# lym01803/FinalProject-LosslessImageCompression

Measured on AMD Instinct MI355X. Metric: encode+decode Mpixels/s (imagenet64, bit-exact round trip), higher is better.
Workload: dtype f32

## Files before the change

### finalproject-losslessimagecompression_amd/csrc/conv3_dx3.hip

```cpp
#include <hip/hip_runtime.h>
#include <stdint.h>
#include <stdlib.h>
#include <string.h>

#include <type_traits>
#include <utility>

#include "idf_cdf.h"
#include "idf_codec_internal.h"
#include "wino_common.h"

#pragma clang fp contract(off)

namespace idf {

typedef float d4 __attribute__((ext_vector_type(4)));
typedef _Float16 e4 __attribute__((ext_vector_type(4)));
typedef _Float16 e8 __attribute__((ext_vector_type(8)));
typedef unsigned int v4u __attribute__((ext_vector_type(4)));
typedef __bf16 b8 __attribute__((ext_vector_type(8)));

struct Dx3Args {
  const uint16_t* xs;
  int64_t P;
// ... 44 lines not shown
#ifndef IDF_DX3_SB
#define IDF_DX3_SB 1
#endif
#ifndef IDF_DX3_DMA0
#define IDF_DX3_DMA0 0
#endif
#ifndef IDF_DX3_DMAS
#define IDF_DX3_DMAS 1
#endif
#ifndef IDF_DX3_STAG
#define IDF_DX3_STAG 0
#endif
#ifndef IDF_DX3_STAMPS
#define IDF_DX3_STAMPS 0
#endif
#ifndef IDF_DX3_STAMP_BLOCK
#define IDF_DX3_STAMP_BLOCK 100
#endif
#if IDF_DX3_STAMPS
__device__ unsigned long long g_dx3_stamp[8][40][4];
__device__ unsigned long long g_dx3_phase[8][6];
#define DX3_PHASE(j, v)                                                                      \
  do {                                                                                      \
    if (blockIdx.x == IDF_DX3_STAMP_BLOCK && lane == 0) g_dx3_phase[wave][(j)] = (v);       \
  } while (0)
#define DX3_STAMP(slab, j)                                                                 \
  do {                                                                                    \
    if (blockIdx.x == IDF_DX3_STAMP_BLOCK && (slab) < 40 && lane == 0)                    \
      g_dx3_stamp[wave][(slab)][(j)] = __builtin_amdgcn_s_memtime();                      \
  } while (0)
#else
#define DX3_STAMP(slab, j) do { } while (0)
#define DX3_PHASE(j, v) do { } while (0)
#endif
#ifndef IDF_DX3_TL
#define IDF_DX3_TL 0
#endif
#if IDF_DX3_TL
__device__ unsigned long long g_dx3_tl[4096][8];
#define DX3_TL(j)                                                                          \
  do {                                                                                    \
    if (tid == 0 && blockIdx.x < 4096) g_dx3_tl[blockIdx.x][(j)] = __builtin_amdgcn_s_memrealtime(); \
  } while (0)
__device__ unsigned long long g_dx3_tlml[1024][16][4];
#define DX3_TLML(li, j)                                                                    \
  do {                                                                                    \
    if (ML && tid == 0 && blockIdx.x < 1024 && (li) < 16)                                 \
      g_dx3_tlml[blockIdx.x][(li)][(j)] = __builtin_amdgcn_s_memrealtime();               \
  } while (0)
#else
#define DX3_TL(j) do { } while (0)
#define DX3_TLML(li, j) do { } while (0)
#endif
#ifndef IDF_DX3_KSPLIT
#define IDF_DX3_KSPLIT 4
#endif
#ifndef IDF_DX3_KSPLIT16
#define IDF_DX3_KSPLIT16 1
#endif
#ifndef IDF_DX3_TWO_MIN
#define IDF_DX3_TWO_MIN 512
#endif
#ifndef IDF_DX3_FORCE1
#define IDF_DX3_FORCE1 0
#endif

#ifndef IDF_DX3_PAIRS
#define IDF_DX3_PAIRS 0
#endif
#ifndef IDF_DX3_PRIO
#define IDF_DX3_PRIO 0
#endif
#ifndef IDF_DX3_PRIO_K
#define IDF_DX3_PRIO_K 4
#endif
#ifndef IDF_DX3_MIX
#define IDF_DX3_MIX 0
#endif
#ifndef IDF_DX3_WAVES
#define IDF_DX3_WAVES 8
#endif
constexpr int kDxWaves = IDF_DX3_WAVES;
constexpr int kDxThreads = 64 * kDxWaves;
constexpr uint32_t kDxInvalid = 0xFFFFFFF0u;
constexpr uint32_t kDxOff = 0x80000000u;
constexpr float kDxInGuard = 32768.0f;
constexpr float kDxOutGuard = 8192.0f;

template <int NF, int WR, int PITCH, int PLANE_KIB, bool BF>
struct Dx3Lds {
  static constexpr int T = WR * kDxWaves / 16;
  static constexpr int HR = WR + 2;
  static constexpr int NS = BF ? 2 * HR - 1 : IDF_DX3_PAIRS ? 3 * HR - 1 + 2 * WR : 5 * HR - 1;
  static constexpr int NPL = BF ? 1 : 2;
  static constexpr int PLANE = PLANE_KIB * 1024;
  static constexpr int SLOTS = PLANE / 32;
  static constexpr int WOFF = T * NPL * PLANE;
  static constexpr int WPART = 9 * NF * 512;
  static constexpr int WST = BF ? (WPART + 1023) / 1024 * 1024 : 2 * WPART;
  static constexpr int STAGE = WOFF + WST;
  static constexpr int ZOFF = 2 * STAGE;
  static constexpr int BOFF = ZOFF + NF * 512;
  static constexpr int HOFF = BOFF + 16 * NF * 16 * 4;
  static constexpr int FOFF = HOFF + 16 * NF * 16 * 4;
  static constexpr int BYTES = FOFF + 16;
  static constexpr int HPIECES = T * NPL * PLANE_KIB;
// ... 80 lines not shown
#pragma unroll
      for (int cls = 0; cls < 16; ++cls) {
        float v = bt[0];
        if (Ly.vtap) {
#pragma unroll
          for (int tap = 0; tap < 9; ++tap) {
            const int dy = tap / 3 - 1, dx = tap % 3 - 1;
            const bool ok = !((dy < 0 && (cls & 1)) || (dy > 0 && (cls & 2)) ||
                              (dx < 0 && (cls & 4)) || (dx > 0 && (cls & 8)));
            v = ok ? v + bt[1 + tap] : v;
          }
          v = cls == 0 ? bt[10] : v;
        }
        btab[cls * NN + tid] = n < g.N ? v : 0.0f;
      }
    }
    if (g.nh > 0) {
#pragma unroll
      for (int i = 0; i < HPER; ++i) {
        const int e = tid + i * kDxThreads, o = e / NN, hn = grp * NN + e - o * NN;
        if (e < NE) htab[e] = (o < g.nh && hn < g.N) ? ht[i] : 0.0f;
      }
    }
  }
};

template <int NF, int WR, int PITCH, int PLANE_KIB, bool BF, bool ML, int WRW = WR>
__device__ __forceinline__ void dx3_block(const Dx3Args& g, const Dx3MLArgs* ml, char* lds) {
  using L = Dx3Lds<NF, WR, PITCH, PLANE_KIB, BF>;
  constexpr bool MIX = WRW != WR;
  constexpr int T = L::T, HR = WRW + 2;
  constexpr int NS = BF ? 2 * HR - 1 : IDF_DX3_PAIRS ? 3 * HR - 1 + 2 * WRW : 5 * HR - 1;
  static_assert(!MIX || (T == 2 && kDxWaves == 8 && !ML && (WRW == WR + 1 || WRW == WR - 1)),
                "mixed rows: two tiles of two SIMD pairs, per-layer launches");
  static_assert(L::WST % 1024 == 0, "weight stage must be whole 1-KiB DMA pieces");
  static_assert(L::BYTES <= 160 * 1024, "LDS");
  static_assert(HR >= 3, "the A-fragment reads of a phase take its last three steps");
  static_assert(IDF_DX3_DMAS == 0 || IDF_DX3_DMA0 + IDF_DX3_STAG + (L::PPW - 1) * IDF_DX3_DMAS < NS,
                "every DMA piece of a slab is issued within the slab's steps");
  int* last_flag = (int*)(lds + L::FOFF);
  const int tid = threadIdx.x, lane = tid & 63;
  const int wave = __builtin_amdgcn_readfirstlane(tid >> 6);
  const int bid = xcd_contiguous(blockIdx.x, gridDim.x);
  const int per_chunk = g.ngroup * g.nblk_tiles;
  const int chunk = udiv_s(bid, per_chunk);
  const int rem = bid - chunk * per_chunk;
  const int grp = udiv_s(rem, g.nblk_tiles);
  const int tb = rem - grp * g.nblk_tiles;
  const int tw = MIX ? (wave & 3) >> 1 : wave / (kDxWaves / T);
  constexpr int WR_OLD = IDF_DX3_MIX == 2 ? WR - 1 : WR + 1;
  const int r0 = MIX ? 2 * WR * (wave & 1) + ((wave & 4) ? WR_OLD : 0) : WR * (wave % (kDxWaves / T));
  d4 hreg[WRW];
  const int nlayers = ML ? ml->nlayers : 1;
  for (int li = 0; li < nlayers; ++li) {
  int tid_o = tid, lane_o = lane, wave_o = wave, tb_o = tb, tw_o = tw, r0_o = r0, grp_o = grp,
      chunk_o = chunk;
  if constexpr (ML) {
    asm volatile("" : "+v"(tid_o), "+v"(lane_o), "+v"(wave_o), "+v"(tb_o), "+v"(tw_o), "+v"(r0_o),
                 "+v"(grp_o), "+v"(chunk_o));
    wave_o = __builtin_amdgcn_readfirstlane(wave_o);
    tb_o = __builtin_amdgcn_readfirstlane(tb_o);
    tw_o = __builtin_amdgcn_readfirstlane(tw_o);
    r0_o = __builtin_amdgcn_readfirstlane(r0_o);
    grp_o = __builtin_amdgcn_readfirstlane(grp_o);
    chunk_o = __builtin_amdgcn_readfirstlane(chunk_o);
  }
  const int tid = tid_o, lane = lane_o, wave = wave_o, tb = tb_o, tw = tw_o, r0 = r0_o,
            grp = grp_o, chunk = chunk_o;
  const int lz = 0;
  DX3_TLML(li, 0);
  Dx3Layer Ly;
  if constexpr (ML) {
    Ly = ml->layer[li];
  } else {
    Ly = Dx3Layer{g.Wt, g.b3, g.vtap, g.bfull, g.out, g.yscale, g.C, g.nslab, g.nchunk,
                  g.chunk_slabs, g.hlast};
  }
  const int tile = tb * T + tw + lz;

  const int64_t plane_b = g.P * 32;
  const int xs_rec = (int)(g.xs_slab < (int64_t)kDxInvalid ? g.xs_slab : (int64_t)kDxInvalid);
  uint32_t pbase[L::PPW];
  int plo[L::PPW];
  bool pok[L::PPW];
  const int s0 = ML ? 0 : chunk * Ly.chunk_slabs;
  const int s1 = ML ? Ly.nslab : min(Ly.nslab, s0 + Ly.chunk_slabs);
  const uint32_t wslab = (uint32_t)(g.ngroup * L::WST);
  const int64_t wbytes = (int64_t)Ly.nslab * wslab;
  const __amdgpu_buffer_rsrc_t wr = __builtin_amdgcn_make_buffer_rsrc(
      (void*)Ly.Wt, 0, (int)(wbytes < (int64_t)kDxInvalid ? wbytes : (int64_t)kDxInvalid), 0x00020000);
  auto dma = [&](int s, int st, int i) {
    if (!pok[i]) return;
    const bool halo = i < L::PH;
    if (halo ? (IDF_DX3_ABLATE & 1) : (IDF_DX3_ABLATE & 4)) return;
    const __amdgpu_buffer_rsrc_t xr = __builtin_amdgcn_make_buffer_rsrc(
        (void*)((const char*)g.xs + (int64_t)s * g.xs_slab), 0, xs_rec, 0x00020000);
    const uint32_t off = pbase[i] + (halo ? 0u : (uint32_t)(s * g.ngroup) * (uint32_t)L::WST);
    __builtin_amdgcn_raw_ptr_buffer_load_lds(halo ? xr : wr,
                                             (dx_lds_ptr_t)(lds + st * L::STAGE + plo[i]), 16,
                                             off, 0, 0, 0);
  };
#pragma unroll
  for (int i = L::PH; i < L::PPW; ++i) {
    const int k = wave + kDxWaves * (i - L::PH);
    pok[i] = k < L::WPIECES;
    plo[i] = pok[i] ? L::WOFF + k * 1024 : 0;
    pbase[i] = pok[i] ? (uint32_t)(grp * L::WST + k * 1024 + lane * 16) : kDxOff;
    if (s1 > s0) dma(s0, 0, i);
  }
  uint32_t forg[T] = {};
  int fu0[T] = {}, fy0[T] = {};
  if constexpr (PITCH == 18) if (g.fastplan) {
#pragma unroll
    for (int t = 0; t < T; ++t) {
      const int tt = tb * T + t;
      const DxTile dtt = dx_tile(g, tt < g.ntiles ? tt : 0);
      const bool tok = tt < g.ntiles && dtt.band < g.B;
      fu0[t] = __builtin_amdgcn_readfirstlane(dtt.u0 - 1);
      fy0[t] = __builtin_amdgcn_readfirstlane(tok ? dtt.u0y - 1 : INT32_MIN / 2);
      forg[t] = __builtin_amdgcn_readfirstlane(
          ((uint32_t)dtt.band * (uint32_t)g.H + (uint32_t)(dtt.u0y - 1)) * (uint32_t)g.Wd + (uint32_t)(dtt.u0 - 1));
    }
  }
#pragma unroll
  for (int i = 0; i < L::PH; ++i) {
    const int k = wave + kDxWaves * i;
    pok[i] = k < L::HPIECES;
    pbase[i] = kDxOff;
    plo[i] = 0;
    if (pok[i]) {
      const int t = k / (L::NPL * PLANE_KIB), pl = (k / PLANE_KIB) % L::NPL, pi = k % PLANE_KIB;
      plo[i] = (t * L::NPL + pl) * L::PLANE + pi * 1024;
      const int slot = 32 * pi + (lane >> 1);
      const int tt = tb * T + t;
      bool fast = false;
      if constexpr (PITCH == 18) fast = g.fastplan != 0;
      if (fast) {
        const int cr = slot / PITCH, cc = slot - cr * PITCH;
        int u0m = fu0[0], y0m = fy0[0];
        uint32_t org = forg[0];
#pragma unroll
        for (int u = 1; u < T; ++u)
          if (t == u) { u0m = fu0[u]; y0m = fy0[u]; org = forg[u]; }
        const bool ok = (uint32_t)(u0m + cc) < (uint32_t)g.Wd && (uint32_t)(y0m + cr) < (uint32_t)g.H &&
                        cr < PITCH;
        if (ok)
          pbase[i] = (uint32_t)pl * (uint32_t)plane_b +
                     (org + (uint32_t)cr * (uint32_t)g.Wd + (uint32_t)cc) * (uint32_t)g.xs_pix +
                     (uint32_t)((lane & 1) * 16);
      } else if (tt < g.ntiles) {
        const DxTile dt = dx_tile(g, tt);
        int ix, x, iy, y;
        bool ok;
        if (g.gut) {
          const int cr = slot / PITCH, cc = slot - cr * PITCH;
          const int u = dt.u0 - 1 + cc, uy = dt.u0y - 1 + cr;
          ix = u >= 0 ? udiv_s(u, g.wp) : 0;
          x = u >= 0 ? u - ix * g.wp : -1;
          iy = uy >= 0 ? udiv_s(uy, g.hp) : 0;
          y = uy >= 0 ? uy - iy * g.hp : -1;
          ok = cr < g.ch && cc < g.segw;
        } else {
          const int sk = g.seg ? udiv_s(slot, g.seg) : 0;
          const int rr = slot - sk * g.seg;
          const int cr = rr / PITCH, cc = rr - cr * PITCH;
          ok = sk < g.nseg && cc < g.segw && cr < g.ch;
          ix = dt.ix0 + sk;
          x = (sk ? 0 : dt.xf0) - 1 + cc;
          const int vy = dt.vy0 + cr;
          iy = udiv_s(vy, g.H + 2);
          y = vy - iy * (g.H + 2) - 1;
        }
        const int b = (dt.band * g.nby + iy) * g.nbx + ix;
        ok = ok && x >= 0 && x < g.Wd && ix < g.nbx && y >= 0 && y < g.H && iy < g.nby && b < g.B;
        if (ok)
          pbase[i] = (uint32_t)(pl * plane_b + ((((int64_t)b * g.H + y) * g.Wd + x) * g.xs_pix) + (lane & 1) * 16);
      }
    }
    if (s1 > s0) dma(s0, 0, i);
  }
  DX3_TL(0);
  if (!ML || li == 0)
    for (int e = tid; e < NF * 512 / 16; e += kDxThreads) *(d4*)(lds + L::ZOFF + 16 * e) = d4{0.f, 0.f, 0.f, 0.f};
  DX3_PHASE(0, __builtin_amdgcn_s_memtime());
  DX3_PHASE(4, __builtin_amdgcn_s_memrealtime());

  const int j = lane & 15, q = lane >> 4;
  const DxTile dt = dx_tile(g, tile < g.ntiles ? tile : 0);
  const int jx = g.xskip ? 3 * (j >> 1) + (j & 1) : j;
  const int uj = dt.u0 + jx;
  const int pw = g.gut ? g.wp : g.Wd;
  const int ixj = udiv_s(uj, pw);
  const int xj = uj - ixj * pw;
  const int kj = ixj - dt.ix0;
  const int colb = g.gut ? jx : kj * g.seg + (kj ? j - (ixj * g.Wd - dt.u0) : j);
  const int uyw = dt.u0y + r0;
  int iyw = udiv_s(uyw, g.H);
  if (iyw > g.nby - 1) iyw = g.nby - 1;
  const int rowb = g.gut ? r0 : uyw + 2 * iyw - dt.vy0;

  const int slot0 = rowb * PITCH + colb;
  const int tb0 = tw * L::NPL * L::PLANE;
  const int oP = tb0 + (q >> 1) * L::PLANE + slot0 * 32 + (q & 1) * 16;
  const int oF = tb0 + slot0 * 32 + (q & 1) * 16 + (q >> 1) * 32;
  const int oG = tb0 + slot0 * 32 + (q & 1) * 16 + 64 + (q >> 1) * PITCH * 32;
  const int oAH = L::WOFF + j * 32 + (q & 1) * 16;
  constexpr int WLO = BF ? 0 : L::WPART;
  const int oAF = L::WOFF + WLO + j * 32 + (q & 1) * 16 + (q >> 1) * NF * 512;
  const int oAG = L::WOFF + WLO + 2 * NF * 512 + j * 32 + (q & 1) * 16 + (q >> 1) * 3 * NF * 512;
  const int oAO = L::WOFF + WLO + 8 * NF * 512 + j * 32 + (q & 1) * 16;
  const int oAHF = L::WOFF + j * 32 + (q & 1) * 16 + (q >> 1) * NF * 512;
  const int oAHG = L::WOFF + 2 * NF * 512 + j * 32 + (q & 1) * 16 + (q >> 1) * 3 * NF * 512;
  const bool zlane = q < 2;
  const char* zO = lds + L::ZOFF + j * 32 + (q & 1) * 16;

  if constexpr (ML) if (li == 0) {
#pragma unroll
    for (int m = 0; m < WRW; ++m) hreg[m] = d4{0.f, 0.f, 0.f, 0.f};
    if (g.nh > 0) {
      const bool lane_ok0 = xj < g.Wd && ixj < g.nbx;
#pragma unroll
      for (int m = 0; m < WRW; ++m) {
        int iy = iyw, y = uyw + m - iyw * g.H;
        if (g.gut) {
          iy = udiv_s(uyw + m, g.hp);
          y = uyw + m - iy * g.hp;
        }
        const int img = (dt.band * g.nby + iy) * g.nbx + ixj;
        const bool ok = lane_ok0 && y < g.H && iy < g.nby && img < g.B;
        if (ok && 4 * q < g.nh) {
          const float* xr = ml->hx + (((int64_t)img * g.H + y) * g.Wd + xj) * ml->hld_x;
          d4 h;
#pragma unroll
          for (int i = 0; i < 4; ++i) h[i] = 4 * q + i < g.nh ? ml->hb[4 * q + i] : 0.0f;
          for (int c = 0; c < ml->hc0; c += 4) {
            const d4 xv = *(const d4*)(xr + c);
#pragma unroll
            for (int i = 0; i < 4; ++i) {
              const int o = 4 * q + i;
              if (o < g.nh) {
                const d4 wv = *(const d4*)(g.hw + (int64_t)o * g.ldhw + c);
#pragma unroll
                for (int k = 0; k < 4; ++k) h[i] = __builtin_fmaf(wv[k], xv[k], h[i]);
              }
            }
          }
          hreg[m] = h;
        }
      }
    }
  }

  Dx3Tables<NF> tabs;
  DX3_PHASE(1, __builtin_amdgcn_s_memtime());
  DX3_TL(1);


  d4 acc[WRW][NF];
#pragma unroll
  for (int m = 0; m < WRW; ++m)
#pragma unroll
    for (int n = 0; n < NF; ++n) acc[m][n] = d4{0.f, 0.f, 0.f, 0.f};

  auto rd = [](const char* p) { return *(const e8*)p; };
  auto mma = [](const e8& a, const e8& bb, d4& c) {
    if (IDF_DX3_ABLATE & 16) c[0] += (float)(a[0] * bb[0]);
    else if constexpr (BF)
      c = __builtin_amdgcn_mfma_f32_16x16x32_bf16(__builtin_bit_cast(b8, a), __builtin_bit_cast(b8, bb),
                                                   c, 0, 0, 0);
    else c = __builtin_amdgcn_mfma_f32_16x16x32_f16(a, bb, c, 0, 0, 0);
  };
  auto rdB = [&](const char* p) -> e8 {
    if (IDF_DX3_ABLATE & 32) return e8{(_Float16)1, (_Float16)(lane & 7), 0, 0, 0, 0, 0, (_Float16)(p == nullptr)};
    return rd(p);
  };
  auto rdA = [&](const char* p) -> e8 {
    if (IDF_DX3_ABLATE & 64) return e8{(_Float16)2, (_Float16)(lane & 3), 0, 0, 0, 0, 0, (_Float16)(p == nullptr)};
    return rd(p);
  };

  constexpr int DB = IDF_DX3_DB, RB = DB + 1;
  e8 Bq[RB];
  e8 AS[2][3][NF];
  e8 AZ[2][NF];
  auto read_B = [&](const char* st, int t) -> e8 {
    if (t < 3 * HR) return rdB(st + oP + ((t % HR) * PITCH + t / HR) * 32);
    if (t < 4 * HR) return rdB(st + oF + (t - 3 * HR) * PITCH * 32);
    return rdB(st + oG + (t - 4 * HR) * PITCH * 32);
  };
  auto read_A = [&](const char* st, int p, int dy, e8 (&A)[NF]) {
#pragma unroll
    for (int n = 0; n < NF; ++n)
      A[n] = p < 3 ? rdA(st + oAH + ((dy * 3 + p) * NF + n) * 512)
                   : rdA(st + oAF + (3 * dy * NF + n) * 512);
  };
  auto mma_rows = [&](const e8 (&A)[3][NF], const e8& Bv, int h) {
#pragma unroll
    for (int dy = 0; dy < 3; ++dy) {
      const int m = h - dy;
      if (m < 0 || m >= WRW) continue;
#pragma unroll
      for (int n = 0; n < NF; ++n) mma(A[dy][n], Bv, acc[m][n]);
    }
  };

  for (int s = s0; s < s1; ++s) {
    const char* cur = lds + ((s - s0) & 1) * L::STAGE;
    DX3_STAMP(s - s0, 0);
    asm volatile("s_waitcnt vmcnt(0) lgkmcnt(0)" ::: "memory");
    if (!(IDF_DX3_ABLATE & 8)) __builtin_amdgcn_s_barrier();
    DX3_STAMP(s - s0, 1);
    if (s == s0) DX3_TL(2);
    if (s == s0) DX3_TLML(li, 1);
    if (s == s0) tabs.load(g, Ly, grp, tid);
    if (s == s0 + 1) tabs.store((float*)(lds + L::BOFF), (float*)(lds + L::HOFF), g, Ly, grp, tid);
    __builtin_amdgcn_sched_barrier(0);
    const bool more = s + 1 < s1;
    const int nst = (s + 1 - s0) & 1;
    auto dma_step = [&](auto tc) {
      constexpr int t = decltype(tc)::value;
      constexpr int ds = IDF_DX3_DMAS > 0 ? IDF_DX3_DMAS : 1;
      auto dma_at = [&](auto dtc) {
        constexpr int dt_ = decltype(dtc)::value;
        if constexpr (IDF_DX3_DMAS == 0 && dt_ == 0) {
          if (more) {
#pragma unroll
            for (int i = 0; i < L::PPW; ++i) dma(s + 1, nst, i);
          }
        } else if constexpr (IDF_DX3_DMAS > 0 && dt_ >= 0 && dt_ % ds == 0 && dt_ / ds < L::PPW) {
          if (more) dma(s + 1, nst, dt_ / ds);
        }
      };
      if (IDF_DX3_STAG == 0 || !(wave & 4)) dma_at(std::integral_constant<int, t - IDF_DX3_DMA0>{});
      else dma_at(std::integral_constant<int, t - IDF_DX3_DMA0 - IDF_DX3_STAG>{});
    };
    if constexpr (BF) {
      auto read_Bf = [&](const char* st, int t) -> e8 {
        if (t < HR) return rdB(st + oF + t * PITCH * 32);
        return rdB(st + oG + (t - HR) * PITCH * 32);
      };
#pragma unroll
      for (int k = 0; k < (DB > 3 ? DB : 3); ++k) {
        if (k < DB) Bq[k] = read_Bf(cur, k);
        if (k < 3) read_A(cur, 3, k, AS[1][k]);
      }
      auto stepb = [&](auto tc) {
        constexpr int t = decltype(tc)::value;
        if (IDF_DX3_SB) __builtin_amdgcn_sched_barrier(0);
        dma_step(tc);
        if constexpr (t == 1 || t == 2) {
#pragma unroll
          for (int n = 0; n < NF; ++n) {
            if (t == 1) AZ[0][n] = rdA(cur + oAG + n * 512);
            else AZ[1][n] = rdA(zlane ? zO + n * 512 : cur + oAO + n * 512);
          }
        }
        if constexpr (t + DB < NS) Bq[(t + DB) % RB] = read_Bf(cur, t + DB);
        const e8& Bv = Bq[t % RB];
        if constexpr (t < HR) {
          mma_rows(AS[1], Bv, t);
        } else {
          constexpr int h = t - HR;
          if constexpr (h < WRW) {
#pragma unroll
            for (int n = 0; n < NF; ++n) mma(AZ[0][n], Bv, acc[h][n]);
          }
          if constexpr (h > 0) {
#pragma unroll
            for (int n = 0; n < NF; ++n) mma(AZ[1][n], Bv, acc[h - 1][n]);
          }
        }
// ... 80 lines not shown
    for (int k = 0; k < (DB > 3 ? DB : 3); ++k) {
      if (k < DB) Bq[k] = read_B(cur, k);
      if (k < 3) read_A(cur, 0, k, AS[0][k]);
    }
    auto step = [&](auto tc) {
      constexpr int t = decltype(tc)::value;
      if (IDF_DX3_SB) __builtin_amdgcn_sched_barrier(0);
      if constexpr (t == 9) DX3_STAMP(s - s0, 2);
      if constexpr (IDF_DX3_PRIO == 1) {
        if (((t & 1) != 0) == ((wave & 4) != 0)) __builtin_amdgcn_s_setprio(1);
        else __builtin_amdgcn_s_setprio(0);
      } else if constexpr (IDF_DX3_PRIO == 2) {
        if (((t / IDF_DX3_PRIO_K) & 1) == ((wave >> 2) & 1)) __builtin_amdgcn_s_setprio(1);
        else __builtin_amdgcn_s_setprio(0);
      } else if constexpr (IDF_DX3_PRIO == 3) {
        if constexpr (t == 0) { if (wave & 4) __builtin_amdgcn_s_setprio(1); }
        if constexpr (t == NS / 2) __builtin_amdgcn_s_setprio(0);
      }
      dma_step(tc);
      if constexpr (t < 3) read_A(cur, 1, t, AS[1][t]);
      if constexpr (t >= HR && t < HR + 3) read_A(cur, 2, t - HR, AS[0][t - HR]);
      if constexpr (t >= 2 * HR && t < 2 * HR + 3) read_A(cur, 3, t - 2 * HR, AS[1][t - 2 * HR]);
      if constexpr (t == 2 * HR + 3 || t == 2 * HR + 4) {
#pragma unroll
        for (int n = 0; n < NF; ++n) {
          if (t == 2 * HR + 3) AZ[0][n] = rdA(cur + oAG + n * 512);
          else AZ[1][n] = rdA(zlane ? zO + n * 512 : cur + oAO + n * 512);
        }
      }
      if constexpr (t + DB < NS) Bq[(t + DB) % RB] = read_B(cur, t + DB);
      const e8& Bv = Bq[t % RB];
      if constexpr (t < 3 * HR) {
        mma_rows(AS[(t / HR) & 1], Bv, t % HR);
      } else if constexpr (t < 4 * HR) {
        mma_rows(AS[1], Bv, t - 3 * HR);
      } else {
        constexpr int h = t - 4 * HR;
        if constexpr (h < WRW) {
#pragma unroll
          for (int n = 0; n < NF; ++n) mma(AZ[0][n], Bv, acc[h][n]);
        }
        if constexpr (h > 0) {
#pragma unroll
          for (int n = 0; n < NF; ++n) mma(AZ[1][n], Bv, acc[h - 1][n]);
        }
      }
    };
    dx_unroll(step, std::make_integer_sequence<int, NS>{});
    DX3_STAMP(s - s0, 3);
  }
  DX3_PHASE(2, __builtin_amdgcn_s_memtime());
  DX3_TL(3);
  DX3_TLML(li, 2);
  if (s1 - s0 <= 1) {
    if (s1 == s0) tabs.load(g, Ly, grp, tid);
    tabs.store((float*)(lds + L::BOFF), (float*)(lds + L::HOFF), g, Ly, grp, tid);
  }
  if (s1 - s0 <= 2) __syncthreads();

  if constexpr (T == 1 && !ML) if (Ly.nchunk > 1) {
    constexpr int FR = kDxWaves * WR * NF;
    const uint32_t pb = (uint32_t)((tb * g.ngroup + grp) * Ly.nchunk) * (FR * 1024u);
    const int64_t pbytes = (int64_t)g.nblk_tiles * g.ngroup * Ly.nchunk * FR * 1024;
    const __amdgpu_buffer_rsrc_t pr = __builtin_amdgcn_make_buffer_rsrc(
        (void*)g.part, 0, (int)(pbytes < (int64_t)kDxInvalid ? pbytes : (int64_t)kDxInvalid), 0x00020000);
    auto poff = [&](int c, int m, int n) -> uint32_t {
      return pb + (uint32_t)((c * FR + (tw * 16 + r0 + m) * NF + n) * 1024 + lane * 16);
    };
#pragma unroll
    for (int m = 0; m < WRW; ++m)
#pragma unroll
      for (int n = 0; n < NF; ++n)
        __builtin_amdgcn_raw_buffer_store_b128(__builtin_bit_cast(v4u, acc[m][n]), pr, poff(chunk, m, n),
                                               0, 16 );
    asm volatile("s_waitcnt vmcnt(0)" ::: "memory");
    __syncthreads();
    if (tid == 0) {
      const uint32_t old = __hip_atomic_fetch_add(g.ctr + tb * g.ngroup + grp, 1u, __ATOMIC_RELAXED,
                                                  __HIP_MEMORY_SCOPE_AGENT);
      const bool last = old == (uint32_t)(Ly.nchunk - 1);
      if (last)
        __hip_atomic_store(g.ctr + tb * g.ngroup + grp, 0u, __ATOMIC_RELAXED, __HIP_MEMORY_SCOPE_AGENT);
      *last_flag = last;
    }
    __syncthreads();
    DX3_TL(6);
    if (!*last_flag) return;
    __builtin_amdgcn_fence(__ATOMIC_ACQUIRE, "wavefront");
    static_assert(IDF_DX3_KSPLIT <= 4, "the reduction holds up to 4 chunks");
    d4 pv[4][WRW][NF];
#pragma unroll
    for (int c = 0; c < 4; ++c)
#pragma unroll
      for (int m = 0; m < WRW; ++m)
#pragma unroll
        for (int n = 0; n < NF; ++n)
          pv[c][m][n] = (c < Ly.nchunk && c != chunk)
                            ? __builtin_bit_cast(d4, __builtin_amdgcn_raw_buffer_load_b128(pr, poff(c, m, n), 0, 16))
                            : acc[m][n];
#pragma unroll
    for (int m = 0; m < WRW; ++m)
#pragma unroll
      for (int n = 0; n < NF; ++n) {
        d4 sum = pv[0][m][n];
#pragma unroll
        for (int c = 1; c < 4; ++c)
          if (c < Ly.nchunk) sum = sum + pv[c][m][n];
        acc[m][n] = sum;
      }
    DX3_TL(4);
  }

  if (tile >= g.ntiles) return;
  const bool lane_ok = xj < g.Wd && ixj < g.nbx;
  const WAct act(g.act, g.slope);
  const float* btab = (const float*)(lds + L::BOFF);
  const float* htab = (const float*)(lds + L::HOFF);
  const bool fh = g.nh > 0;
  bool out_ok = true;
  const int zr = (Ly.C + g.N + 15) / 16 * 16, zend = zr < 16 * g.nslab_xs ? zr : 16 * g.nslab_xs;
  const bool lastg = grp == g.ngroup - 1;
  char* xsb = (char*)g.xs;
  int r_img[WRW], r_y[WRW];
  int64_t r_pix[WRW];
  bool r_ok[WRW];
#pragma unroll
  for (int m = 0; m < WRW; ++m) {
    int iy = iyw, y = uyw + m - iyw * g.H;
    if (g.gut) {
      iy = udiv_s(uyw + m, g.hp);
      y = uyw + m - iy * g.hp;
    }
    r_img[m] = (dt.band * g.nby + iy) * g.nbx + ixj;
    r_y[m] = y;
    r_ok[m] = lane_ok && y < g.H && iy < g.nby && r_img[m] < g.B;
    r_pix[m] = ((int64_t)r_img[m] * g.H + y) * g.Wd + xj;
  }
  d4 hprev[WRW];
#pragma unroll
  for (int m = 0; m < WRW; ++m) {
    hprev[m] = d4{0.f, 0.f, 0.f, 0.f};
    if constexpr (ML) hprev[m] = hreg[m];
    else if (fh && r_ok[m] && 4 * q < g.nh) hprev[m] = *(const d4*)(g.hacc + r_pix[m] * 16 + 4 * q);
  }
  auto outputs = [&](auto tanh_c) {
    constexpr bool TANH = decltype(tanh_c)::value;
#pragma unroll
    for (int m = 0; m < WRW; ++m) {
      const bool row_ok = r_ok[m];
      if (!row_ok && !fh) continue;
      const int cls = bias_class(r_y[m], xj, g.H, g.Wd);
      const int64_t pix = r_pix[m];
      float* dst = Ly.out + pix * g.ldo;
      d4 bv[NF];
#pragma unroll
      for (int n = 0; n < NF; ++n) bv[n] = *(const d4*)(btab + cls * (NF * 16) + 16 * n + 4 * q);
#pragma unroll
      for (int n = 0; n <= NF; ++n) {
        if (n == NF && !lastg) break;
        const int nl = 16 * n + 4 * q;
        const int n0 = 16 * grp * NF + nl;
        d4 v = d4{0.f, 0.f, 0.f, 0.f};
        if (n < NF) {
          const bool live = n0 < g.N;
#pragma unroll
          for (int k = 0; k < 4; ++k) {
            const float t = acc[m][n][k] * Ly.yscale + bv[n][k];
            if constexpr (TANH) v[k] = wact(t, g.act, g.slope);
            else v[k] = act(t);
            if (!BF) out_ok = out_ok && (!(live && row_ok) || fabsf(v[k]) < kDxOutGuard);
          }
          if (live && row_ok && !g.skip_f32) {
            if (n0 + 4 <= g.N) {
              *(d4*)(dst + n0) = v;
            } else {
#pragma unroll
              for (int k = 0; k < 4; ++k)
                if (n0 + k < g.N) dst[n0 + k] = v[k];
            }
          }
#pragma unroll
          for (int k = 0; k < 4; ++k) v[k] = n0 + k < g.N ? v[k] : 0.0f;
          acc[m][n] = v;
        }
        const int c = Ly.C + n0;
        if (row_ok && !(IDF_DX3_ABLATE & 128) && c < zend) {
// ... 44 lines not shown
        const float mine = q < 2 ? hp[m][i] : hp[m][8 + i];
        const float give = q < 2 ? hp[m][8 + i] : hp[m][i];
        r8[i] = mine + __shfl_xor(give, 32);
      }
#pragma unroll
      for (int i = 0; i < 4; ++i) {
        const float mine = (q & 1) ? r8[4 + i] : r8[i];
        const float give = (q & 1) ? r8[i] : r8[4 + i];
        r4[i] = mine + __shfl_xor(give, 16);
      }
      if (r_ok[m] && 4 * q < g.nh) {
        const int64_t pix = r_pix[m];
        d4* ap = (d4*)(g.hacc + pix * 16 + 4 * q);
        const d4 prev = hprev[m];
        d4 hv;
#pragma unroll
        for (int i = 0; i < 4; ++i) hv[i] = prev[i] + r4[i];
        if (!Ly.hlast) {
          if constexpr (ML) hreg[m] = hv;
          else *ap = hv;
        } else {
          const int b_img = r_img[m];
          const int64_t hw_ = (int64_t)g.H * g.Wd, rem = (int64_t)r_y[m] * g.Wd + xj;
#pragma unroll
          for (int i = 0; i < 4; ++i) {
            const int o = 4 * q + i;
            if (o >= g.nh) break;
            const float vv = hv[i];
            if (g.hmode == IDF_EPI_COUPLE_ADD || g.hmode == IDF_EPI_COUPLE_SUB) {
              const float r = __builtin_rintf(vv * 256.0f) / 256.0f;
              const float bsv = g.hbase[pix * g.hld_base + o];
              g.hout[pix * g.hld_out + o] = g.hmode == IDF_EPI_COUPLE_ADD ? bsv + r : bsv - r;
            } else if (g.hmode == IDF_EPI_PRIOR) {
              if (o < g.hn_mean) {
                g.hmean[((int64_t)b_img * g.hn_mean + o) * hw_ + rem] = vv;
              } else {
                const int64_t oi = ((int64_t)b_img * g.hn_mean + (o - g.hn_mean)) * hw_ + rem;
                g.hlogs[oi] = vv;
                g.hscale[oi] = expf_glibc(vv);
              }
            } else {
              g.hout[pix * g.hld_out + o] = vv;
            }
          }
        }
      }
    }
  }
  if (!out_ok && g.flag) atomicOr(g.flag, 1u);
  DX3_TL(5);
  DX3_PHASE(3, __builtin_amdgcn_s_memtime());
  DX3_PHASE(5, __builtin_amdgcn_s_memrealtime());
  if constexpr (ML) {
    asm volatile("s_waitcnt vmcnt(0) lgkmcnt(0)" ::: "memory");
    __builtin_amdgcn_s_barrier();
    DX3_TLML(li, 3);
  }
  }
}

template <int NF, int WR, int PITCH, int PLANE_KIB, bool BF>
__global__ void __launch_bounds__(kDxThreads, 1) conv3_dx3_kernel(Dx3Args g) {
  __shared__ __attribute__((aligned(16))) char lds[Dx3Lds<NF, WR, PITCH, PLANE_KIB, BF>::BYTES];
  if constexpr (IDF_DX3_MIX && !BF && WR * kDxWaves == 32 && WR >= 2) {
    constexpr int D = IDF_DX3_MIX == 2 ? -1 : 1;
    if (threadIdx.x < 256) dx3_block<NF, WR, PITCH, PLANE_KIB, BF, false, WR + D>(g, nullptr, lds);
    else dx3_block<NF, WR, PITCH, PLANE_KIB, BF, false, WR - D>(g, nullptr, lds);
  } else {
    dx3_block<NF, WR, PITCH, PLANE_KIB, BF, false>(g, nullptr, lds);
  }
}

template <int NF, int PITCH, int PLANE_KIB, bool BF>
__global__ void __launch_bounds__(kDxThreads, 1) conv3_dx3_block_kernel(Dx3Args g, Dx3MLArgs ml) {
  __shared__ __attribute__((aligned(16))) char lds[Dx3Lds<NF, 16 / kDxWaves, PITCH, PLANE_KIB, BF>::BYTES];
  dx3_block<NF, 16 / kDxWaves, PITCH, PLANE_KIB, BF, true>(g, &ml, lds);
}

__device__ __forceinline__ void dx3_head_init_pixel(int64_t p, int32_t C0, const float* __restrict__ x,
                                                    int64_t ld_x, const float* __restrict__ w,
                                                    int32_t ldw, const float* __restrict__ bias,
                                                    int32_t nh, float* __restrict__ acc) {
  float h[16];
#pragma unroll
  for (int o = 0; o < 16; ++o) h[o] = o < nh ? bias[o] : 0.0f;
  const float* xr = x + p * ld_x;
  for (int c = 0; c < C0; c += 4) {
    const d4 xv = *(const d4*)(xr + c);
#pragma unroll
    for (int o = 0; o < 16; ++o) {
      if (o >= nh) break;
      const d4 wv = *(const d4*)(w + (int64_t)o * ldw + c);
#pragma unroll
      for (int k = 0; k < 4; ++k) h[o] = __builtin_fmaf(wv[k], xv[k], h[o]);
    }
  }
  d4* ap = (d4*)(acc + p * 16);
#pragma unroll
  for (int i = 0; i < 4; ++i) ap[i] = d4{h[4 * i], h[4 * i + 1], h[4 * i + 2], h[4 * i + 3]};
}

struct Dx3HeadInit {
  const float* w;
  int32_t ldw;
  const float* bias;
  int32_t nh;
  float* acc;
};
__global__ void __launch_bounds__(256) dx3_split_cols_kernel(int64_t P, int32_t c0, int32_t c1,
// ... 550 lines not shown
```

### finalproject-losslessimagecompression_amd/csrc/flow_kernels.hip

```cpp
#include <hip/hip_runtime.h>
#include <stdint.h>

#include <algorithm>
#include <vector>

#include "idf_cdf.h"
#include "idf_codec_internal.h"

#pragma clang fp contract(off)

namespace idf {

typedef float floatx4 __attribute__((ext_vector_type(4)));

enum { MODE_DENSE = 0, MODE_CONV3 = 1 };
enum { EPI_STORE = 0, EPI_ACT = 1, EPI_COUPLE_ADD = 2, EPI_COUPLE_SUB = 3, EPI_PRIOR = 4,
       EPI_ACT_FOLD = 5 };

struct GemmArgs {
  int64_t P;
  int32_t K;
  int32_t N;
  const float* A;
  int64_t lda;
// ... 645 lines not shown
}

extern "C" int64_t idf_dense_block_dx3_tmp_bytes(const IdfDenseBlock* blk, int32_t B, int32_t H,
                                                  int32_t W) {
  BlockPlan pl;
  return block_args_ok(blk, B, H, W) && !dense_block_plan(blk, B, H, W, true, &pl) ? pl.bytes : -1;
}

extern "C" int idf_dense_block_plan(const IdfDenseBlock* blk, int32_t B, int32_t H, int32_t W,
                                    int32_t with_head, int32_t out[IDF_BLOCK_PLAN_N]) {
  if (!out) return IDF_ERR_ARG;
  for (int i = 0; i < IDF_BLOCK_PLAN_N; ++i) out[i] = 0;
  if (!block_args_ok(blk, B, H, W)) return IDF_ERR_ARG;
  BlockPlan pl;
  if (int rc = dense_block_plan(blk, B, H, W, with_head != 0, &pl)) return rc;
  out[IDF_BLOCK_PLAN_FUSED] = pl.fused;
  out[IDF_BLOCK_PLAN_HEAD] = pl.head;
  out[IDF_BLOCK_PLAN_HEAD_INIT] = pl.head_init;
  out[IDF_BLOCK_PLAN_N_DX3] = pl.n_dx3;
  out[IDF_BLOCK_PLAN_CONV_LAUNCHES] = pl.conv_launches;
  out[IDF_BLOCK_PLAN_SETUP_LAUNCHES] = pl.setup_launches;
  out[IDF_BLOCK_PLAN_HEAD_LAUNCHES] = pl.head_launches;
  for (int i = 0; i < blk->depth; ++i) {
    out[IDF_BLOCK_PLAN_KIND0 + i] = pl.kind[i];
    if (pl.wx3_first[i]) out[IDF_BLOCK_PLAN_WX3_FIRST] |= (int32_t)(1u << i);
  }
  return IDF_OK;
}

static int dense_block_run_fused(void* stream, const IdfDenseBlock* blk, const BlockPlan& pl,
                                 int32_t B, int32_t H, int32_t W, float* feat, int64_t ld_feat,
                                 uint16_t* xs, const IdfDx3Head* hd, IdfTimer* timer) {
  const bool dxb = pl.copy == COPY_DXB;
  const int64_t P = (int64_t)B * H * W;
  int32_t C[16];
  const uint16_t* w[16];
  float ys[16];
  const float *b3[16], *vt[16], *bfu[16];
  double fl = 0.0;
  for (int i = 0; i < blk->depth; ++i) {
    C[i] = blk->k_in[i];
    w[i] = dxb ? blk->dxb_w[i] : blk->dx3_w[i];
    ys[i] = dxb ? 1.0f : blk->dx3_yscale[i];
    b3[i] = blk->b3[i];
    vt[i] = blk->vtap[i];
    bfu[i] = blk->bfull[i];
    fl += 2.0 * P * 9.0 * blk->c_real[i] * blk->g_real[i];
  }
  IdfDx3BlockDesc d = {};
  d.bf = dxb ? 1 : 0;
  d.B = B; d.H = H; d.W = W; d.nlayers = blk->depth; d.N = blk->g_pad; d.nft = pl.dx3_nft;
  d.ldv = blk->ldv; d.act = blk->act; d.nslab_xs = pl.nslab_xs; d.slope = blk->slope;
  d.xs = xs; d.C = C; d.w = w; d.yscale = ys; d.b3 = b3;
  d.vtap = blk->vtap[0] ? vt : nullptr; d.bfull = blk->vtap[0] ? bfu : nullptr;
  d.feat = feat; d.ld_feat = ld_feat; d.flag = dxb ? nullptr : blk->range_flag;
  d.head = hd;
  d.hx = feat; d.hld_x = ld_feat; d.hc0 = blk->k_in[0]; d.hb = blk->bh;
  timer_mark(timer, (hipStream_t)stream, IDF_TAG_CONV3X3, fl, true);
  const int rc = idf_dx3_block_launch(stream, &d);
  timer_mark(timer, (hipStream_t)stream, 0, 0, false);
  return rc;
}

static int dense_block_run(void* stream, const IdfDenseBlock* blk, int32_t B, int32_t H, int32_t W,
                           float* feat, int64_t ld_feat, float* tmp, int64_t ld_tmp,
                           const IdfHeadOut* head, IdfTimer* timer) {
  if (!blk || blk->depth < 0 || blk->depth > IDF_MAX_DEPTH) return IDF_ERR_ARG;
  const int depth = blk->depth;
  const int64_t P = (int64_t)B * H * W;
  if (ld_feat < blk->k_in[depth] || ld_tmp < blk->k_in[depth]) return IDF_ERR_ARG;
  hipStream_t s = (hipStream_t)stream;
  BlockPlan pl;
  if (int rc = dense_block_plan(blk, B, H, W, head != nullptr, &pl)) return rc;
  const int64_t tmp_floats = P * ld_tmp;
  const bool direct = pl.copy == COPY_DX3_SPLIT || pl.copy == COPY_DXB;
  if (pl.sh16 > tmp_floats || pl.bytes > tmp_floats * 4 || (direct && (uintptr_t)tmp % 256))
    return IDF_ERR_WORKSPACE;
  uint16_t* const xs = (uint16_t*)tmp;
  float* const ws = tmp + pl.sh16;
  char* const dws = (char*)tmp + pl.off;
  float* const hacc = pl.head == IDF_PLAN_HEAD_FUSED ? (float*)((char*)tmp + pl.hoff) : nullptr;
  const int c0 = blk->k_in[0];
  uint32_t* const ctr = pl.need > 0 ? (uint32_t*)dws : nullptr;
  const int32_t nctr =
      pl.need > 0 ? (int32_t)(idf_conv3x3_dx3_counter_bytes(B, H, W, blk->g_pad) / 4) : 0;
  int rc = IDF_OK;
  switch (pl.copy) {
    case COPY_BF16_SHADOW:
      rc = idf_f32_to_bf16_cols(stream, P, c0, (c0 + 7) / 8 * 8, feat, ld_feat, xs, pl.ld16);
      break;
    case COPY_DXB:
      rc = idf_dxb_cols(stream, P, 0, c0, feat, ld_feat, xs, pl.nslab_xs, ctr, nctr);
      break;
    case COPY_DX3_SPLIT:
      rc = pl.head_init == IDF_HEAD_INIT_IN_SPLIT
               ? idf_dx3_split_cols_head(stream, P, c0, feat, ld_feat, xs, pl.nslab_xs,
                                         blk->range_flag, ctr, nctr, blk->wh, blk->ldwh, blk->bh,
                                         blk->n_head, hacc)
               : idf_dx3_split_cols(stream, P, 0, c0, feat, ld_feat, xs, pl.nslab_xs,
                                    blk->range_flag, ctr, nctr);
      break;
  }
  if (rc) return rc;
  if (pl.head_init == IDF_HEAD_INIT_OWN_LAUNCH) {
    rc = idf_dx3_head_init(stream, P, c0, feat, ld_feat, blk->wh, blk->ldwh, blk->bh, blk->n_head,
                           hacc);
    if (rc) return rc;
// ... 258 lines not shown
```

Baseline: 21.43.

## Prefetch next layer's weights and carry address state across fused dx3 layers

In the multi-layer fused dx3 block kernel, the first weight slab of the next layer is issued into the free LDS stage during the current layer's epilogue. The end-of-layer wait and barrier are skipped when that prefetch is in flight, and the stage parity is carried across layers. Per-lane DMA bases and LDS offsets are computed once on the first layer and reused afterwards, so later layers skip recomputing them. This aims to hide the weight-load latency at layer boundaries, at the cost of more fragile synchronisation: the prefetched stage must not overlap data the epilogue still reads. The host now always passes the vtap/bfull arrays.

```diff
diff --git a/finalproject-losslessimagecompression_amd/csrc/conv3_dx3.hip b/finalproject-losslessimagecompression_amd/csrc/conv3_dx3.hip
--- a/finalproject-losslessimagecompression_amd/csrc/conv3_dx3.hip
+++ b/finalproject-losslessimagecompression_amd/csrc/conv3_dx3.hip
@@ -120,6 +120,12 @@
 #define DX3_TL(j) do { } while (0)
 #define DX3_TLML(li, j) do { } while (0)
 #endif
+#ifndef IDF_DX3_ML_OVERLAP
+#define IDF_DX3_ML_OVERLAP 1
+#endif
+#ifndef IDF_DX3_ML_CARRY
+#define IDF_DX3_ML_CARRY 1
+#endif
 #ifndef IDF_DX3_KSPLIT
 #define IDF_DX3_KSPLIT 4
 #endif
@@ -306,6 +312,13 @@
   const int r0 = MIX ? 2 * WR * (wave & 1) + ((wave & 4) ? WR_OLD : 0) : WR * (wave % (kDxWaves / T));
   d4 hreg[WRW];
   const int nlayers = ML ? ml->nlayers : 1;
+  int sp = 0;
+  bool pre = false;
+  uint32_t pbase[L::PPW];
+  int plo[L::PPW];
+  bool pok[L::PPW];
+  int oP = 0, oF = 0, oG = 0, oAH = 0, oAF = 0, oAG = 0, oAO = 0, oAHF = 0, oAHG = 0;
+  int xj = 0, ixj = 0, uyw = 0, iyw = 0, band = 0;
   for (int li = 0; li < nlayers; ++li) {
   int tid_o = tid, lane_o = lane, wave_o = wave, tb_o = tb, tw_o = tw, r0_o = r0, grp_o = grp,
       chunk_o = chunk;
@@ -334,33 +347,34 @@
 
   const int64_t plane_b = g.P * 32;
   const int xs_rec = (int)(g.xs_slab < (int64_t)kDxInvalid ? g.xs_slab : (int64_t)kDxInvalid);
-  uint32_t pbase[L::PPW];
-  int plo[L::PPW];
-  bool pok[L::PPW];
   const int s0 = ML ? 0 : chunk * Ly.chunk_slabs;
   const int s1 = ML ? Ly.nslab : min(Ly.nslab, s0 + Ly.chunk_slabs);
   const uint32_t wslab = (uint32_t)(g.ngroup * L::WST);
   const int64_t wbytes = (int64_t)Ly.nslab * wslab;
   const __amdgpu_buffer_rsrc_t wr = __builtin_amdgcn_make_buffer_rsrc(
       (void*)Ly.Wt, 0, (int)(wbytes < (int64_t)kDxInvalid ? wbytes : (int64_t)kDxInvalid), 0x00020000);
-  auto dma = [&](int s, int st, int i) {
+  auto dma_w = [&](const __amdgpu_buffer_rsrc_t& wres, int s, int st, int i) {
     if (!pok[i]) return;
     const bool halo = i < L::PH;
     if (halo ? (IDF_DX3_ABLATE & 1) : (IDF_DX3_ABLATE & 4)) return;
     const __amdgpu_buffer_rsrc_t xr = __builtin_amdgcn_make_buffer_rsrc(
         (void*)((const char*)g.xs + (int64_t)s * g.xs_slab), 0, xs_rec, 0x00020000);
     const uint32_t off = pbase[i] + (halo ? 0u : (uint32_t)(s * g.ngroup) * (uint32_t)L::WST);
-    __builtin_amdgcn_raw_ptr_buffer_load_lds(halo ? xr : wr,
+    __builtin_amdgcn_raw_ptr_buffer_load_lds(halo ? xr : wres,
                                              (dx_lds_ptr_t)(lds + st * L::STAGE + plo[i]), 16,
                                              off, 0, 0, 0);
   };
+  auto dma = [&](int s, int st, int i) { dma_w(wr, s, st, i); };
+  const bool dma0 = s1 > s0 && !pre;
+  const int j = lane & 15, q = lane >> 4;
+  if (!ML || li == 0 || !IDF_DX3_ML_CARRY) {
 #pragma unroll
   for (int i = L::PH; i < L::PPW; ++i) {
     const int k = wave + kDxWaves * (i - L::PH);
     pok[i] = k < L::WPIECES;
     plo[i] = pok[i] ? L::WOFF + k * 1024 : 0;
     pbase[i] = pok[i] ? (uint32_t)(grp * L::WST + k * 1024 + lane * 16) : kDxOff;
-    if (s1 > s0) dma(s0, 0, i);
+    if (dma0) dma(s0, sp, i);
   }
   uint32_t forg[T] = {};
   int fu0[T] = {}, fy0[T] = {};
@@ -431,7 +445,7 @@
           pbase[i] = (uint32_t)(pl * plane_b + ((((int64_t)b * g.H + y) * g.Wd + x) * g.xs_pix) + (lane & 1) * 16);
       }
     }
-    if (s1 > s0) dma(s0, 0, i);
+    if (dma0) dma(s0, sp, i);
   }
   DX3_TL(0);
   if (!ML || li == 0)
@@ -439,32 +453,37 @@
   DX3_PHASE(0, __builtin_amdgcn_s_memtime());
   DX3_PHASE(4, __builtin_amdgcn_s_memrealtime());
 
-  const int j = lane & 15, q = lane >> 4;
   const DxTile dt = dx_tile(g, tile < g.ntiles ? tile : 0);
+  band = dt.band;
   const int jx = g.xskip ? 3 * (j >> 1) + (j & 1) : j;
   const int uj = dt.u0 + jx;
   const int pw = g.gut ? g.wp : g.Wd;
-  const int ixj = udiv_s(uj, pw);
-  const int xj = uj - ixj * pw;
+  ixj = udiv_s(uj, pw);
+  xj = uj - ixj * pw;
   const int kj = ixj - dt.ix0;
   const int colb = g.gut ? jx : kj * g.seg + (kj ? j - (ixj * g.Wd - dt.u0) : j);
-  const int uyw = dt.u0y + r0;
-  int iyw = udiv_s(uyw, g.H);
+  uyw = dt.u0y + r0;
+  iyw = udiv_s(uyw, g.H);
   if (iyw > g.nby - 1) iyw = g.nby - 1;
   const int rowb = g.gut ? r0 : uyw + 2 * iyw - dt.vy0;
 
   const int slot0 = rowb * PITCH + colb;
   const int tb0 = tw * L::NPL * L::PLANE;
-  const int oP = tb0 + (q >> 1) * L::PLANE + slot0 * 32 + (q & 1) * 16;
-  const int oF = tb0 + slot0 * 32 + (q & 1) * 16 + (q >> 1) * 32;
-  const int oG = tb0 + slot0 * 32 + (q & 1) * 16 + 64 + (q >> 1) * PITCH * 32;
-  const int oAH = L::WOFF + j * 32 + (q & 1) * 16;
+  oP = tb0 + (q >> 1) * L::PLANE + slot0 * 32 + (q & 1) * 16;
+  oF = tb0 + slot0 * 32 + (q & 1) * 16 + (q >> 1) * 32;
+  oG = tb0 + slot0 * 32 + (q & 1) * 16 + 64 + (q >> 1) * PITCH * 32;
+  oAH = L::WOFF + j * 32 + (q & 1) * 16;
   constexpr int WLO = BF ? 0 : L::WPART;
-  const int oAF = L::WOFF + WLO + j * 32 + (q & 1) * 16 + (q >> 1) * NF * 512;
-  const int oAG = L::WOFF + WLO + 2 * NF * 512 + j * 32 + (q & 1) * 16 + (q >> 1) * 3 * NF * 512;
-  const int oAO = L::WOFF + WLO + 8 * NF * 512 + j * 32 + (q & 1) * 16;
-  const int oAHF = L::WOFF + j * 32 + (q & 1) * 16 + (q >> 1) * NF * 512;
-  const int oAHG = L::WOFF + 2 * NF * 512 + j * 32 + (q & 1) * 16 + (q >> 1) * 3 * NF * 512;
+  oAF = L::WOFF + WLO + j * 32 + (q & 1) * 16 + (q >> 1) * NF * 512;
+  oAG = L::WOFF + WLO + 2 * NF * 512 + j * 32 + (q & 1) * 16 + (q >> 1) * 3 * NF * 512;
+  oAO = L::WOFF + WLO + 8 * NF * 512 + j * 32 + (q & 1) * 16;
+  oAHF = L::WOFF + j * 32 + (q & 1) * 16 + (q >> 1) * NF * 512;
+  oAHG = L::WOFF + 2 * NF * 512 + j * 32 + (q & 1) * 16 + (q >> 1) * 3 * NF * 512;
+  } else {
+#pragma unroll
+    for (int i = 0; i < L::PPW; ++i)
+      if (dma0) dma(s0, sp, i);
+  }
   const bool zlane = q < 2;
   const char* zO = lds + L::ZOFF + j * 32 + (q & 1) * 16;
 
@@ -480,7 +499,7 @@
           iy = udiv_s(uyw + m, g.hp);
           y = uyw + m - iy * g.hp;
         }
-        const int img = (dt.band * g.nby + iy) * g.nbx + ixj;
+        const int img = (band * g.nby + iy) * g.nbx + ixj;
         const bool ok = lane_ok0 && y < g.H && iy < g.nby && img < g.B;
         if (ok && 4 * q < g.nh) {
           const float* xr = ml->hx + (((int64_t)img * g.H + y) * g.Wd + xj) * ml->hld_x;
@@ -559,7 +578,7 @@
   };
 
   for (int s = s0; s < s1; ++s) {
-    const char* cur = lds + ((s - s0) & 1) * L::STAGE;
+    const char* cur = lds + ((s - s0 + sp) & 1) * L::STAGE;
     DX3_STAMP(s - s0, 0);
     asm volatile("s_waitcnt vmcnt(0) lgkmcnt(0)" ::: "memory");
     if (!(IDF_DX3_ABLATE & 8)) __builtin_amdgcn_s_barrier();
@@ -570,7 +589,7 @@
     if (s == s0 + 1) tabs.store((float*)(lds + L::BOFF), (float*)(lds + L::HOFF), g, Ly, grp, tid);
     __builtin_amdgcn_sched_barrier(0);
     const bool more = s + 1 < s1;
-    const int nst = (s + 1 - s0) & 1;
+    const int nst = (s + 1 - s0 + sp) & 1;
     auto dma_step = [&](auto tc) {
       constexpr int t = decltype(tc)::value;
       constexpr int ds = IDF_DX3_DMAS > 0 ? IDF_DX3_DMAS : 1;
@@ -757,6 +776,20 @@
   DX3_PHASE(2, __builtin_amdgcn_s_memtime());
   DX3_TL(3);
   DX3_TLML(li, 2);
+  bool pre_next = false;
+  if constexpr (ML && IDF_DX3_ML_OVERLAP) {
+    if (li + 1 < nlayers && Ly.C >= 16 && s1 - s0 >= 2) {
+      const Dx3Layer& Nx = ml->layer[li + 1];
+      const int64_t nbytes = (int64_t)Nx.nslab * wslab;
+      const __amdgpu_buffer_rsrc_t wn = __builtin_amdgcn_make_buffer_rsrc(
+          (void*)Nx.Wt, 0, (int)(nbytes < (int64_t)kDxInvalid ? nbytes : (int64_t)kDxInvalid), 0x00020000);
+      if (Nx.nslab >= 2) {
+#pragma unroll
+        for (int i = 0; i < L::PPW; ++i) dma_w(wn, 0, (sp + s1 - s0) & 1, i);
+        pre_next = true;
+      }
+    }
+  }
   if (s1 - s0 <= 1) {
     if (s1 == s0) tabs.load(g, Ly, grp, tid);
     tabs.store((float*)(lds + L::BOFF), (float*)(lds + L::HOFF), g, Ly, grp, tid);
@@ -836,7 +869,7 @@
       iy = udiv_s(uyw + m, g.hp);
       y = uyw + m - iy * g.hp;
     }
-    r_img[m] = (dt.band * g.nby + iy) * g.nbx + ixj;
+    r_img[m] = (band * g.nby + iy) * g.nbx + ixj;
     r_y[m] = y;
     r_ok[m] = lane_ok && y < g.H && iy < g.nby && r_img[m] < g.B;
     r_pix[m] = ((int64_t)r_img[m] * g.H + y) * g.Wd + xj;
@@ -987,9 +1020,15 @@
   DX3_PHASE(3, __builtin_amdgcn_s_memtime());
   DX3_PHASE(5, __builtin_amdgcn_s_memrealtime());
   if constexpr (ML) {
-    asm volatile("s_waitcnt vmcnt(0) lgkmcnt(0)" ::: "memory");
-    __builtin_amdgcn_s_barrier();
+    if (!pre_next) {
+      asm volatile("s_waitcnt vmcnt(0) lgkmcnt(0)" ::: "memory");
+      __builtin_amdgcn_s_barrier();
+    }
     DX3_TLML(li, 3);
+    if constexpr (IDF_DX3_ML_OVERLAP) {
+      sp = (sp + s1 - s0) & 1;
+      pre = pre_next;
+    }
   }
   }
 }
diff --git a/finalproject-losslessimagecompression_amd/csrc/flow_kernels.hip b/finalproject-losslessimagecompression_amd/csrc/flow_kernels.hip
--- a/finalproject-losslessimagecompression_amd/csrc/flow_kernels.hip
+++ b/finalproject-losslessimagecompression_amd/csrc/flow_kernels.hip
@@ -721,7 +721,7 @@
   d.B = B; d.H = H; d.W = W; d.nlayers = blk->depth; d.N = blk->g_pad; d.nft = pl.dx3_nft;
   d.ldv = blk->ldv; d.act = blk->act; d.nslab_xs = pl.nslab_xs; d.slope = blk->slope;
   d.xs = xs; d.C = C; d.w = w; d.yscale = ys; d.b3 = b3;
-  d.vtap = blk->vtap[0] ? vt : nullptr; d.bfull = blk->vtap[0] ? bfu : nullptr;
+  d.vtap = vt; d.bfull = bfu;
   d.feat = feat; d.ld_feat = ld_feat; d.flag = dxb ? nullptr : blk->range_flag;
   d.head = hd;
   d.hx = feat; d.hld_x = ld_feat; d.hc0 = blk->k_in[0]; d.hb = blk->bh;
```

After: 21.49, median of 2. No clear change (+0.3%).
